# snipsco/sda

Hardware: AMD Instinct MI355X
Metric: share-gen + clerk-sum elements/sec (mod q) (higher is better)
Workload: dtype u64

## Files before the change

sda_amd/csrc/varint_kernels.hip:

```cpp
#include <hip/hip_runtime.h>
#include <stdint.h>

#include "capi_internal.hpp"
#include "drbg_quad.hpp"
#include "kernels.hpp"
#include "modarith.hpp"
#include "sbox_primitives.hpp"

namespace sda {

static constexpr int kVT = 256;
static constexpr int kVals = 8;
static constexpr int kBytes = 16;

__device__ __forceinline__ uint64_t zigzag(int64_t v) { return ((uint64_t)v << 1) ^ (uint64_t)(v >> 63); }
__device__ __forceinline__ uint32_t varint_len(uint64_t zz) {
    const uint32_t x = (64u - (uint32_t)__clzll(zz | 1ull)) + 6u;
    return (x * 37u) >> 8;
}

__device__ __forceinline__ uint32_t block_exscan(uint32_t v, uint32_t* lds_waves, uint32_t* total) {
    const int lane = threadIdx.x & 63, wave = threadIdx.x >> 6;
    uint32_t incl = v;
#pragma unroll
// ... 711 lines not shown
            rs.next_group(sink);
            if (rs.done()) { rs.close(status); live = false; }
        }
        if ((threadIdx.x & 63) == 0) cols[wave] = live ? rs.col : len;
        __syncthreads();
        if (window_flush<kCombWaves>(lo32, hi32, sink, cols, len)) break;
    }
}

static constexpr int kKsStride = 66;
static constexpr int kKsTile = 16 * kKsStride;

struct XSalsaBytes {
    uint32_t key[8], n0, n1;
    uint32_t* ks;
    __device__ __forceinline__ void open(const SboxState& st, uint32_t* tile) {
        const int lane = threadIdx.x & 63;
#pragma unroll
        for (int i = 0; i < 8; ++i) key[i] = st.subkey[i];
        n0 = st.n0; n1 = st.n1;
        ks = tile;
        uint32_t b[16];
        sbx::salsa20_block(b, key, n0, n1, 0);
        if (lane == 0) {
#pragma unroll
            for (int w = 0; w < 16; ++w) ks[w * kKsStride + 64] = b[w];
        }
    }
    __device__ __forceinline__ void begin_group(uint64_t j0) {
        const int lane = threadIdx.x & 63;
        __builtin_amdgcn_fence(__ATOMIC_ACQ_REL, "wavefront");
        __builtin_amdgcn_wave_barrier();
        if (lane < 16) ks[lane * kKsStride] = ks[lane * kKsStride + 64];
        __builtin_amdgcn_fence(__ATOMIC_ACQ_REL, "wavefront");
        __builtin_amdgcn_wave_barrier();
        uint32_t b[16];
        sbx::salsa20_block(b, key, n0, n1, 16 * j0 + 1 + (uint64_t)lane);
#pragma unroll
        for (int w = 0; w < 16; ++w) ks[w * kKsStride + 1 + lane] = b[w];
        __builtin_amdgcn_fence(__ATOMIC_ACQ_REL, "wavefront");
        __builtin_amdgcn_wave_barrier();
    }
    __device__ __forceinline__ void apply(uint4& cur, int d, bool ciphertext) const {
        const uint32_t p = 2u + 64u * (uint32_t)d + (threadIdx.x & 63u);
        const uint32_t* k = ks + (p & 3u) * 4u * kKsStride + (p >> 2);
        if (ciphertext) {
            cur.x ^= k[0]; cur.y ^= k[kKsStride]; cur.z ^= k[2 * kKsStride]; cur.w ^= k[3 * kKsStride];
        }
    }
    __device__ __forceinline__ uint32_t byte_at(uint8_t c, uint64_t m) const {
        const uint64_t sp = m + 32;
        uint32_t b[16];
        sbx::salsa20_block(b, key, n0, n1, sp >> 6);
        uint32_t word = 0;
#pragma unroll
        for (int w = 0; w < 16; ++w) word = ((uint32_t)(sp >> 2) & 15u) == (uint32_t)w ? b[w] : word;
        return (c ^ (word >> (8 * (uint32_t)(sp & 3)))) & 0xFFu;
    }
};

__device__ __forceinline__ bool sealed_row_open(RowStreamT<XSalsaBytes>& rs, const uint8_t* __restrict__ boxes, uint64_t slot,
                                                const uint64_t* __restrict__ row_bytes, uint64_t max_box,
                                                const SboxState* __restrict__ states, uint64_t r, uint64_t len,
                                                uint32_t* __restrict__ status, uint8_t* tile, uint32_t* kstream) {
    const bool lead = (threadIdx.x & 63) == 0;
    const uint64_t have = row_bytes[r];
    if (!(have >= 48 && have <= max_box && have <= slot && !states[r].bad)) return false;
    const uint64_t a = r * slot + 48, b = r * slot + have;
    if (len == 0) { if (a != b && lead) atomicOr(status, SDA_VARINT_ROW_COUNT); return false; }
    if (a == b) { if (lead) atomicOr(status, SDA_VARINT_UNTERMINATED); return false; }
    rs.crypt.open(states[r], kstream);
    if (rs.crypt.byte_at(boxes[b - 1], b - 1 - a) & 0x80u) { if (lead) atomicOr(status, SDA_VARINT_UNTERMINATED); return false; }
    rs.open(boxes, a, b, len, tile);
    return true;
}

template <int kCombWaves>
__global__ __launch_bounds__(kCombWaves * 64) void sealed_stream_combine_kernel(
    const uint8_t* __restrict__ boxes, uint64_t slot, const uint64_t* __restrict__ row_bytes, uint64_t max_box,
    const SboxState* __restrict__ states, uint64_t rows, uint64_t len, uint64_t* __restrict__ acc_lo,
    int64_t* __restrict__ acc_hi, uint32_t* __restrict__ status) {
    __shared__ __attribute__((aligned(16))) uint8_t tiles[kCombWaves][kStreamTile];
    __shared__ uint32_t kstream[kCombWaves][kKsTile];
    __shared__ unsigned long long lo32[kCombWindow], hi32[kCombWindow];
    __shared__ uint64_t cols[kCombWaves];
    const int wave = threadIdx.x >> 6;
    const bool lead = (threadIdx.x & 63) == 0;
    const uint64_t r = (uint64_t)blockIdx.x * kCombWaves + wave;
    for (int i = threadIdx.x; i < kCombWindow; i += kCombWaves * 64) { lo32[i] = 0; hi32[i] = 0; }
    RowStreamT<XSalsaBytes> rs;
    bool live = r < rows && sealed_row_open(rs, boxes, slot, row_bytes, max_box, states, r, len, status, tiles[wave], kstream[wave]);
    WindowSink sink{lo32, hi32, 0, acc_lo, acc_hi};
    __syncthreads();
    for (;;) {
        if (live) {
            rs.next_group(sink);
            if (rs.done()) { rs.close(status); live = false; }
        }
        if (lead) cols[wave] = live ? rs.col : len;
        __syncthreads();
        if (window_flush<kCombWaves>(lo32, hi32, sink, cols, len)) break;
    }
}

static constexpr int kCoefLds = 16;

struct WeightedSink {
    WindowSink win;
    const uint64_t* coef;
    uint32_t k;
    uint64_t batches, m, mu, pinv;
    __device__ __forceinline__ void operator()(uint64_t b, int64_t v) const {
        if (b >= batches) return;
        const uint64_t x = canon_i64(v, m, mu);
        const uint64_t c = b * k;
        for (uint32_t s = 0; s < k; ++s) win(c + s, (int64_t)mont_redc(mul64x64(coef[s], x), m, pinv));
    }
};

template <int kCombWaves, bool kLds>
__global__ __launch_bounds__(kCombWaves * 64) void sealed_stream_weighted_kernel(
    const uint8_t* __restrict__ boxes, uint64_t slot, const uint64_t* __restrict__ row_bytes, uint64_t max_box,
    const SboxState* __restrict__ states, uint64_t rows, uint64_t len, uint64_t first_pos, WeightedJob J,
    uint64_t* __restrict__ acc_lo, int64_t* __restrict__ acc_hi, uint32_t* __restrict__ status) {
    __shared__ __attribute__((aligned(16))) uint8_t tiles[kCombWaves][kStreamTile];
    __shared__ uint32_t kstream[kCombWaves][kKsTile];
    __shared__ unsigned long long lo32[kCombWindow], hi32[kCombWindow];
    __shared__ uint64_t cols[kCombWaves];
    __shared__ uint32_t alive[kCombWaves];
    __shared__ uint64_t coefs[kLds ? kCombWaves : 1][kCoefLds];
    const int wave = __builtin_amdgcn_readfirstlane(threadIdx.x >> 6), lane = threadIdx.x & 63;
    const bool lead = lane == 0;
    const uint64_t r = (uint64_t)blockIdx.x * kCombWaves + wave;
    const uint64_t total = J.batches * J.k;
    for (int i = threadIdx.x; i < kCombWindow; i += kCombWaves * 64) { lo32[i] = 0; hi32[i] = 0; }
    const uint64_t* coef = J.Rt + (first_pos + (r < rows ? r : 0)) * J.k;
    if (kLds) {
        if (r < rows && (uint32_t)lane < J.k) coefs[wave][lane] = coef[lane];
        coef = coefs[wave];
    }
    RowStreamT<XSalsaBytes> rs;
    bool live = r < rows && sealed_row_open(rs, boxes, slot, row_bytes, max_box, states, r, len, status, tiles[wave], kstream[wave]);
    WeightedSink sink{{lo32, hi32, 0, acc_lo, acc_hi}, coef, J.k, J.batches, J.m, J.mu, J.pinv};
    __syncthreads();
    for (;;) {
        if (live) {
            rs.next_group(sink);
            if (rs.done()) { rs.close(status); live = false; }
        }
        if (lead) {
            cols[wave] = live && rs.col < J.batches ? rs.col * J.k : total;
            alive[wave] = live;
        }
        __syncthreads();
        uint32_t any = 0;
#pragma unroll
        for (int w = 0; w < kCombWaves; ++w) any |= alive[w];
        const bool flushed = window_flush<kCombWaves>(lo32, hi32, sink.win, cols, total);
        if (flushed && !any) break;
    }
}

__global__ __launch_bounds__(kVT) void weighted_rows_kernel(const int64_t* __restrict__ shares, uint64_t row_stride, uint32_t rows,
                                                            uint64_t first_pos, WeightedJob J, uint64_t* __restrict__ acc_lo,
                                                            int64_t* __restrict__ acc_hi, uint32_t e_per_group) {
    const uint64_t b = (uint64_t)blockIdx.x * kVT + threadIdx.x;
    if (b >= J.batches) return;
    const uint32_t e0 = blockIdx.y * e_per_group, e1 = e0 + e_per_group < J.k ? e0 + e_per_group : J.k;
    for (uint32_t e = e0; e < e1; ++e) {
        U128 acc{0, 0};
        uint32_t since = 0;
        for (uint32_t c = 0; c < rows; ++c) {
            const uint64_t v = canon_i64(shares[(uint64_t)c * row_stride + b], J.m, J.mu);
            mac128(acc, J.Rt[(first_pos + c) * J.k + e], v);
            if (++since == 4) { mont_acc_condsub(acc, J.m); since = 0; }
        }
        mont_acc_condsub(acc, J.m);
        const uint64_t o = b * J.k + e;
        acc_atomic_add(acc_lo + o, acc_hi + o, mont_redc(acc, J.m, J.pinv), 0);
    }
}

__global__ __launch_bounds__(kVT) void transpose_u64_kernel(const uint64_t* __restrict__ in, uint64_t* __restrict__ out, uint32_t k,
                                                            uint32_t n) {
    const uint64_t i = (uint64_t)blockIdx.x * kVT + threadIdx.x;
    if (i >= (uint64_t)k * n) return;
    const uint64_t pos = i / k, s = i - pos * k;
    out[i] = in[s * n + pos];
}

struct EncXSalsa {
    uint32_t key[8], n0, n1;
    uint32_t* ks;
    uint64_t base;
    __device__ __forceinline__ void fill() {
        const int lane = threadIdx.x & 63;
        __builtin_amdgcn_fence(__ATOMIC_ACQ_REL, "wavefront");
        __builtin_amdgcn_wave_barrier();
        uint32_t b[16];
        sbx::salsa20_block(b, key, n0, n1, base + (uint64_t)lane);
#pragma unroll
        for (int w = 0; w < 16; ++w) ks[w * kKsStride + lane] = b[w];
        __builtin_amdgcn_fence(__ATOMIC_ACQ_REL, "wavefront");
        __builtin_amdgcn_wave_barrier();
    }
    __device__ __forceinline__ void open(const SboxState& st, uint32_t* tile) {
#pragma unroll
        for (int i = 0; i < 8; ++i) key[i] = st.subkey[i];
        n0 = st.n0; n1 = st.n1;
        ks = tile;
        base = 0;
        fill();
    }
    __device__ __forceinline__ bool ends_before(uint64_t unit_end) const { return unit_end + 2 > 4 * (base + 64); }
    __device__ __forceinline__ bool holds(uint64_t u) const { return u + 2 < 4 * (base + 64); }
    __device__ __forceinline__ void refill() { base += 64; fill(); }
    __device__ __forceinline__ void apply(uint4& v, uint64_t u) const {
        const uint32_t p = (uint32_t)(u + 2 - 4 * base);
        const uint32_t* k = ks + (p & 3u) * 4u * kKsStride + (p >> 2);
        v.x ^= k[0]; v.y ^= k[kKsStride]; v.z ^= k[2 * kKsStride]; v.w ^= k[3 * kKsStride];
    }
};

__global__ __launch_bounds__(kStreamWaves * 64) void varint_seal_stream_kernel(VarintRows R, uint8_t* __restrict__ boxes, uint64_t slot,
                                                                               const SboxState* __restrict__ states,
                                                                               uint64_t* __restrict__ msg_bytes) {
    __shared__ __attribute__((aligned(16))) uint8_t tiles[kStreamWaves][kEncTile];
    __shared__ uint32_t kstream[kStreamWaves][kKsTile];
    const int wave = threadIdx.x >> 6;
    const uint64_t r = (uint64_t)blockIdx.x * kStreamWaves + wave;
    if (r >= R.rows) return;
    if (states[r].bad) { if ((threadIdx.x & 63) == 0) msg_bytes[r] = 0; return; }
    EncXSalsa crypt;
    crypt.open(states[r], kstream[wave]);
    LoadValues vals;
    vals.open(R.values + r * R.row_stride, R.len);
    encode_row(vals, R.len, r, boxes + r * slot + 48, tiles[wave], msg_bytes, crypt);
}

template <int ROUNDS>
struct ShareValues {
    static constexpr int kDepth = 1;
    const ShareJob& J;
    const int64_t* __restrict__ sp;
    const uint64_t* __restrict__ row;
    uint64_t stream;
    uint32_t T, draw;
    QuadCol qc;
    __device__ __forceinline__ ShareValues(const ShareJob& J_, uint32_t c, uint64_t p) : J(J_) {
        sp = J.secrets + p * J.secrets_stride;
        stream = J.first_participant + p;
        qc = quad_col(J.key);
        T = J.additive ? J.n - 1 : J.t;
        const uint32_t direct = J.additive ? J.n - 1 : J.direct_rows;
        draw = c < direct ? c : T;
        row = J.additive || c < direct ? nullptr : J.M + (uint64_t)(c - direct) * (J.k + J.t);
    }
    __device__ __forceinline__ void get(int, uint64_t j, int64_t& x, int64_t& y) {
        const uint64_t pair = j * (kEncVals / 2) + (threadIdx.x & 63u);
        const uint64_t b0 = 2 * pair;
        const uint64_t m = J.mod.m, mu = J.mod.mu;
        uint64_t r0, r1;
        if (draw < T) {
            drbg_pair<ROUNDS>(J.key, qc, stream, pair, T, draw, J.mod, r0, r1);
            x = (int64_t)r0; y = (int64_t)r1;
            return;
        }
        if (J.additive) {
            uint64_t s0 = b0 < J.len ? canon_i64(sp[b0], m, mu) : 0;
            uint64_t s1 = b0 + 1 < J.len ? canon_i64(sp[b0 + 1], m, mu) : 0;
            for (uint32_t i = 0; i < T; ++i) {
                drbg_pair<ROUNDS>(J.key, qc, stream, pair, T, i, J.mod, r0, r1);
                s0 = submod(s0, r0, m);
                s1 = submod(s1, r1, m);
            }
            x = (int64_t)s0; y = (int64_t)s1;
            return;
        }
        U128 a0{0, 0}, a1{0, 0};
        uint32_t since = 0;
        const uint64_t e0 = b0 * J.k, e1 = e0 + J.k;
        for (uint32_t i = 0; i < J.k; ++i) {
            const uint64_t v0 = e0 + i < J.len ? canon_i64(sp[e0 + i], m, mu) : 0;
            const uint64_t v1 = e1 + i < J.len ? canon_i64(sp[e1 + i], m, mu) : 0;
            const uint64_t cf = row[i];
            mac128(a0, cf, v0);
            mac128(a1, cf, v1);
            if (++since == 4) { mont_acc_condsub(a0, J.mont.p); mont_acc_condsub(a1, J.mont.p); since = 0; }
        }
        for (uint32_t i = 0; i < T; ++i) {
            drbg_pair<ROUNDS>(J.key, qc, stream, pair, T, i, J.mod, r0, r1);
            const uint64_t cf = row[J.k + i];
            mac128(a0, cf, r0);
            mac128(a1, cf, r1);
            if (++since == 4) { mont_acc_condsub(a0, J.mont.p); mont_acc_condsub(a1, J.mont.p); since = 0; }
        }
        mont_acc_condsub(a0, J.mont.p);
        mont_acc_condsub(a1, J.mont.p);
        x = (int64_t)mont_redc(a0, J.mont.p, J.mont.pinv);
        y = (int64_t)mont_redc(a1, J.mont.p, J.mont.pinv);
    }
};

template <int ROUNDS>
__global__ __launch_bounds__(kStreamWaves * 64) void share_seal_stream_kernel(ShareJob J, uint32_t by_rows, uint8_t* __restrict__ boxes,
                                                                              uint64_t slot, const SboxState* __restrict__ states,
                                                                              uint64_t* __restrict__ msg_bytes) {
    __shared__ __attribute__((aligned(16))) uint8_t tiles[kStreamWaves][kEncTile];
    __shared__ uint32_t kstream[kStreamWaves][kKsTile];
    const int wave = __builtin_amdgcn_readfirstlane(threadIdx.x >> 6);
    uint64_t c, p;
    if (by_rows) {
        const uint64_t r = (uint64_t)blockIdx.x * kStreamWaves + wave;
        c = r / J.participants; p = r - c * J.participants;
    } else {
        const uint32_t groups = (J.n + kStreamWaves - 1) / kStreamWaves;
        p = blockIdx.x / groups;
        c = (uint64_t)(blockIdx.x - p * groups) * kStreamWaves + wave;
    }
    if (c >= J.n || p >= J.participants) return;
    const uint64_t r = c * J.participants + p;
    if (states[r].bad) { if ((threadIdx.x & 63) == 0) msg_bytes[r] = 0; return; }
    EncXSalsa crypt;
    crypt.open(states[r], kstream[wave]);
    ShareValues<ROUNDS> vals(J, (uint32_t)c, p);
    encode_row(vals, J.batches, r, boxes + r * slot + 48, tiles[wave], msg_bytes, crypt);
}

template <int ROUNDS>
struct MaskValues {
    static constexpr int kDepth = 1;
    const MaskJob& J;
    const int64_t* sp;
    int64_t* mp;
    uint64_t stream;
    bool vec;
    QuadCol qc;
    __device__ __forceinline__ MaskValues(const MaskJob& J_, uint64_t p) : J(J_) {
        sp = J.secrets + p * J.secrets_stride;
        mp = J.masked + p * J.masked_stride;
        stream = J.first_participant + p;
        vec = ((((uintptr_t)sp) | ((uintptr_t)mp)) & 15u) == 0;
        qc = quad_col(J.key);
    }
    __device__ __forceinline__ void get(int, uint64_t j, int64_t& x, int64_t& y) {
        typedef long long ll2v __attribute__((ext_vector_type(2)));
        const uint64_t pair = j * (kEncVals / 2) + (threadIdx.x & 63u);
        const uint64_t b0 = 2 * pair;
        const bool two = vec && b0 + 1 < J.len;
        const bool one0 = !two && b0 < J.len, one1 = !two && b0 + 1 < J.len;
        long long s0 = 0, s1 = 0;
        if (two) {
            const ll2v v = __builtin_nontemporal_load(reinterpret_cast<const ll2v*>(sp + b0));
            s0 = v.x; s1 = v.y;
        }
        if (one0) s0 = __builtin_nontemporal_load(reinterpret_cast<const long long*>(sp + b0));
        if (one1) s1 = __builtin_nontemporal_load(reinterpret_cast<const long long*>(sp + b0 + 1));
        __builtin_amdgcn_sched_barrier(0);
        uint64_t r0, r1;
        drbg_pair<ROUNDS>(J.key, qc, stream, pair, 1, 0, J.mod, r0, r1);
        const uint64_t m = J.mod.m, mu = J.mod.mu;
        const long long m0 = (long long)addmod(canon_i64(s0, m, mu), r0, m);
        const long long m1 = (long long)addmod(canon_i64(s1, m, mu), r1, m);
        if (two) {
            ll2v v;
            v.x = m0; v.y = m1;
            __builtin_nontemporal_store(v, reinterpret_cast<ll2v*>(mp + b0));
        }
        if (one0) __builtin_nontemporal_store(m0, reinterpret_cast<long long*>(mp + b0));
        if (one1) __builtin_nontemporal_store(m1, reinterpret_cast<long long*>(mp + b0 + 1));
        x = (int64_t)r0; y = (int64_t)r1;
    }
};

template <int ROUNDS>
__global__ __launch_bounds__(kStreamWaves * 64) void mask_seal_stream_kernel(MaskJob J, uint8_t* __restrict__ boxes, uint64_t slot,
                                                                             const SboxState* __restrict__ states,
                                                                             uint64_t* __restrict__ msg_bytes) {
    __shared__ __attribute__((aligned(16))) uint8_t tiles[kStreamWaves][kEncTile];
    __shared__ uint32_t kstream[kStreamWaves][kKsTile];
    const int wave = __builtin_amdgcn_readfirstlane(threadIdx.x >> 6);
    const uint64_t p = (uint64_t)blockIdx.x * kStreamWaves + wave;
    if (p >= J.participants) return;
    if (states[p].bad) { if ((threadIdx.x & 63) == 0) msg_bytes[p] = 0; return; }
    EncXSalsa crypt;
    crypt.open(states[p], kstream[wave]);
    MaskValues<ROUNDS> vals(J, p);
    encode_row(vals, J.len, p, boxes + p * slot + 48, tiles[wave], msg_bytes, crypt);
}

static constexpr int kSumVals = kVT * kVals;
static constexpr int kSumStage = 64 + kSumVals * 10;
static constexpr int kSumKsBlocks = kSumStage / 64;
static constexpr int kSumKsStride = 17;

size_t sum_seal_blocks(size_t len) { return (size_t)((len + kSumVals - 1) / kSumVals); }

__global__ __launch_bounds__(kVT) void sum_len_kernel(SumRows S, uint32_t* __restrict__ block_bytes) {
    __shared__ uint32_t waves[kVT / 64];
    const uint64_t job = blockIdx.y;
    const uint64_t* lo = S.acc_lo + job * S.len;
    const int64_t* hi = S.acc_hi + job * S.len;
    const uint64_t i0 = (uint64_t)blockIdx.x * kSumVals + threadIdx.x;
    uint32_t sum = 0;
    for (int u = 0; u < kVals; ++u) {
        const uint64_t i = i0 + (uint64_t)u * kVT;
        if (i < S.len) sum += varint_len(zigzag((int64_t)mod_i128(lo[i], hi[i], S.m, S.mu)));
    }
    uint32_t total;
    (void)block_exscan(sum, waves, &total);
    if (threadIdx.x == 0) block_bytes[job * gridDim.x + blockIdx.x] = total;
}

__global__ __launch_bounds__(kVT) void sum_seal_wide_kernel(SumRows S, const uint64_t* __restrict__ block_off, uint8_t* __restrict__ boxes,
                                                            uint64_t slot, const SboxState* __restrict__ states,
                                                            uint64_t* __restrict__ msg_bytes) {
    __shared__ uint32_t waves[kVT / 64];
    __shared__ __attribute__((aligned(16))) uint8_t stage[kSumStage + 16];
    __shared__ uint32_t ks[kSumKsBlocks * kSumKsStride];
    const uint64_t job = blockIdx.y, blk = blockIdx.x, n_blk = gridDim.x;
    const bool last = blk + 1 == n_blk;
    const SboxState& st = states[job];
    if (st.bad) { if (last && threadIdx.x == 0) msg_bytes[job] = 0; return; }
    const uint64_t off = block_off[job * n_blk + blk] - block_off[job * n_blk];
    const uint32_t pad = (uint32_t)((off + 32) & 63u);
    const uint64_t ks0 = (off + 32) >> 6;
    const uint64_t* lo = S.acc_lo + job * S.len;
    const int64_t* hi = S.acc_hi + job * S.len;
    const uint64_t i0 = blk * kSumVals + (uint64_t)threadIdx.x * kVals;
    uint64_t zz[kVals];
    uint32_t ln[kVals];
    uint32_t sum = 0;
    for (int k = 0; k < kVals; ++k) {
        zz[k] = 0; ln[k] = 0;
        if (i0 + k < S.len) {
            zz[k] = zigzag((int64_t)mod_i128(lo[i0 + k], hi[i0 + k], S.m, S.mu));
            ln[k] = varint_len(zz[k]);
            sum += ln[k];
        }
    }
    uint32_t total;
    uint32_t pos = pad + block_exscan(sum, waves, &total);
#pragma unroll
    for (int k = 0; k < kVals; ++k) {
        if (ln[k]) {
            uint64_t n = zz[k];
            for (uint32_t b = 0; b + 1 < ln[k]; ++b) { stage[pos++] = (uint8_t)(0x80u | (n & 0x7Fu)); n >>= 7; }
            stage[pos++] = (uint8_t)n;
        }
    }
    if (total) {
        uint32_t key[8];
#pragma unroll
        for (int i = 0; i < 8; ++i) key[i] = st.subkey[i];
        const uint32_t n_ks = (pad + total + 63u) >> 6;
        for (uint32_t i = threadIdx.x; i < n_ks; i += kVT) {
            uint32_t b[16];
            sbx::salsa20_block(b, key, st.n0, st.n1, ks0 + i);
#pragma unroll
            for (int w = 0; w < 16; ++w) ks[i * kSumKsStride + w] = b[w];
        }
    }
    __syncthreads();
    uint32_t* stage32 = reinterpret_cast<uint32_t*>(stage);
    const uint32_t n_words = total ? (pad + total + 3u) >> 2 : 0u;
    for (uint32_t x = threadIdx.x; x < n_words; x += kVT) stage32[x] ^= ks[(x >> 4) * kSumKsStride + (x & 15u)];
    __syncthreads();
    uint8_t* dst = boxes + job * slot + 48 + off;
    const uint32_t head = (uint32_t)((4u - (uint32_t)((uintptr_t)dst & 3u)) & 3u);
    const uint32_t h = head < total ? head : total;
    if (threadIdx.x < h) dst[threadIdx.x] = stage[pad + threadIdx.x];
    const uint32_t n_dw = (total - h) >> 2;
    uint32_t* dst32 = reinterpret_cast<uint32_t*>(dst + h);
    for (uint32_t d = threadIdx.x; d < n_dw; d += kVT) {
        const uint32_t byte = pad + h + 4u * d;
        const uint32_t w0 = stage32[byte >> 2], w1 = stage32[(byte >> 2) + 1];
        dst32[d] = __builtin_amdgcn_alignbyte(w1, w0, byte & 3u);
    }
    const uint32_t done = h + 4u * n_dw;
    if (threadIdx.x < total - done) dst[done + threadIdx.x] = stage[pad + done + threadIdx.x];
    if (last && threadIdx.x == 0) msg_bytes[job] = off + total;
}

static inline uint64_t vceil(uint64_t a, uint64_t b) { return (a + b - 1) / b; }

size_t varint_encode_blocks(size_t rows, size_t len) { return (size_t)vceil((uint64_t)rows * len, kVT * kVals); }
size_t varint_decode_blocks(size_t n_bytes) { return (size_t)vceil(n_bytes, kVT * kBytes); }

hipError_t launch_varint_lengths(const VarintRows& R, uint32_t* d_block_bytes, hipStream_t s) {
    const size_t nb = varint_encode_blocks(R.rows, R.len);
    if (nb == 0) return hipSuccess;
    if (nb > 0xFFFFFFFFull / kVT) return hipErrorInvalidConfiguration;
    varint_len_kernel<<<dim3((unsigned)nb), dim3(kVT), 0, s>>>(R, d_block_bytes);
    return hipGetLastError();
}

size_t scan_aux_entries(size_t n) { return (n + 1023) / 1024 + 1; }

hipError_t launch_scan_u32(const uint32_t* d_in, uint64_t* d_out, size_t n, uint64_t* d_total, uint64_t* d_aux,
                           hipStream_t s) {
    const size_t m = (n + 1023) / 1024;
    if (m == 0) return hipMemsetAsync(d_total, 0, 8, s);
    if (m > 0xFFFFFFFFull / 1024) return hipErrorInvalidConfiguration;
    scan_chunks_kernel<<<dim3((unsigned)m), dim3(1024), 0, s>>>(d_in, d_out, d_aux, n);
    scan_totals_kernel<<<dim3(1), dim3(1024), 0, s>>>(d_aux, m, d_total);
    scan_add_kernel<<<dim3((unsigned)m), dim3(1024), 0, s>>>(d_out, d_aux, n);
    return hipGetLastError();
}

hipError_t launch_varint_write(const VarintRows& R, const uint64_t* d_block_off, uint8_t* d_out, uint64_t* d_row_offsets,
                               hipStream_t s) {
    const size_t nb = varint_encode_blocks(R.rows, R.len);
    if (nb == 0) return hipSuccess;
    varint_write_kernel<<<dim3((unsigned)nb), dim3(kVT), 0, s>>>(R, d_block_off, d_out, d_row_offsets);
    return hipGetLastError();
}

hipError_t launch_varint_count(const uint8_t* d_bytes, size_t n_bytes, uint32_t* d_block_counts, hipStream_t s) {
    const size_t nb = varint_decode_blocks(n_bytes);
    if (nb == 0) return hipSuccess;
    if (nb > 0xFFFFFFFFull / kVT) return hipErrorInvalidConfiguration;
    varint_count_kernel<<<dim3((unsigned)nb), dim3(kVT), 0, s>>>(d_bytes, n_bytes, d_block_counts);
    return hipGetLastError();
}

hipError_t launch_varint_decode(const uint8_t* d_bytes, size_t n_bytes, const uint64_t* d_block_val_off, size_t rows,
                                size_t len, size_t row_stride, int64_t* d_out, uint32_t* d_status, hipStream_t s) {
    const size_t nb = varint_decode_blocks(n_bytes);
    if (nb == 0) return hipSuccess;
    varint_decode_kernel<<<dim3((unsigned)nb), dim3(kVT), 0, s>>>(d_bytes, n_bytes, d_block_val_off, rows, len, row_stride,
                                                                  d_out, d_status);
    return hipGetLastError();
}

hipError_t launch_varint_stream_decode(const uint8_t* d_bytes, size_t n_bytes, const RowRanges& d_offsets, size_t rows,
                                       size_t len, size_t row_stride, int64_t* d_out, uint32_t* d_status, hipStream_t s) {
    if (rows == 0) return hipSuccess;
    varint_stream_decode_kernel<<<dim3((unsigned)vceil(rows, kStreamWaves)), dim3(kStreamWaves * 64), 0, s>>>(
        d_bytes, n_bytes, d_offsets, rows, len, row_stride, d_out, d_status);
    return hipGetLastError();
}

hipError_t launch_varint_stream_encode(const VarintRows& R, uint8_t* d_out, size_t slot_bytes, uint64_t* d_row_bytes,
                                       hipStream_t s) {
    if (R.rows == 0) return hipSuccess;
    varint_stream_encode_kernel<<<dim3((unsigned)vceil(R.rows, kStreamWaves)), dim3(kStreamWaves * 64), residency_pad_bytes(knob(KNOB_WIRE_WG_PER_CU), 8192), s>>>(
        R, d_out, slot_bytes, d_row_bytes);
    return hipGetLastError();
}

hipError_t launch_varint_seal_stream(const VarintRows& R, uint8_t* d_boxes, size_t slot_bytes, const SboxState* d_states,
                                     uint64_t* d_msg_bytes, hipStream_t s) {
    if (R.rows == 0) return hipSuccess;
    const uint64_t groups = vceil(R.rows, kStreamWaves);
    if (groups > 0x7FFFFFFFull) return hipErrorInvalidConfiguration;
    varint_seal_stream_kernel<<<dim3((unsigned)groups), dim3(kStreamWaves * 64), 0, s>>>(R, d_boxes, slot_bytes, d_states, d_msg_bytes);
    return hipGetLastError();
}

static bool sum_grid(const SumRows& S, dim3* grid) {
    const uint64_t nb = sum_seal_blocks(S.len);
    if (S.jobs > 65535 || nb * S.jobs > 0xFFFFFFFFull / kVT) return false;
    *grid = dim3((unsigned)nb, (unsigned)S.jobs);
    return true;
}

hipError_t launch_sum_lengths(const SumRows& S, uint32_t* d_block_bytes, hipStream_t s) {
    if (S.jobs == 0 || S.len == 0) return hipSuccess;
    dim3 grid;
    if (!sum_grid(S, &grid)) return hipErrorInvalidConfiguration;
    sum_len_kernel<<<grid, dim3(kVT), 0, s>>>(S, d_block_bytes);
    return hipGetLastError();
}

hipError_t launch_sum_seal_wide(const SumRows& S, const uint64_t* d_block_off, uint8_t* d_boxes, size_t slot_bytes,
                                const SboxState* d_states, uint64_t* d_msg_bytes, hipStream_t s) {
    if (S.jobs == 0) return hipSuccess;
    if (S.len == 0) return hipMemsetAsync(d_msg_bytes, 0, S.jobs * sizeof(uint64_t), s);
    dim3 grid;
    if (!sum_grid(S, &grid)) return hipErrorInvalidConfiguration;
    sum_seal_wide_kernel<<<grid, dim3(kVT), 0, s>>>(S, d_block_off, d_boxes, slot_bytes, d_states, d_msg_bytes);
    return hipGetLastError();
}

hipError_t launch_share_seal_stream(const ShareJob& J, int rounds, uint8_t* d_boxes, size_t slot_bytes, const SboxState* d_states,
                                    uint64_t* d_msg_bytes, hipStream_t s) {
    if (J.participants == 0 || J.n == 0) return hipSuccess;
    const bool by_rows = knob(KNOB_GENSEAL_BY_ROWS) != 0;
    const uint64_t groups = by_rows ? vceil((uint64_t)J.n * J.participants, kStreamWaves) : vceil(J.n, kStreamWaves) * (uint64_t)J.participants;
    if (groups > 0x7FFFFFFFull) return hipErrorInvalidConfiguration;
    const dim3 grid((unsigned)groups), block(kStreamWaves * 64);
    switch (rounds) {
        case 20: share_seal_stream_kernel<20><<<grid, block, 0, s>>>(J, by_rows, d_boxes, slot_bytes, d_states, d_msg_bytes); break;
        case 12: share_seal_stream_kernel<12><<<grid, block, 0, s>>>(J, by_rows, d_boxes, slot_bytes, d_states, d_msg_bytes); break;
        case 8: share_seal_stream_kernel<8><<<grid, block, 0, s>>>(J, by_rows, d_boxes, slot_bytes, d_states, d_msg_bytes); break;
        default: return hipErrorInvalidValue;
    }
    return hipGetLastError();
}

hipError_t launch_mask_seal_stream(const MaskJob& J, int rounds, uint8_t* d_boxes, size_t slot_bytes, const SboxState* d_states,
                                   uint64_t* d_msg_bytes, hipStream_t s) {
    if (J.participants == 0) return hipSuccess;
    const uint64_t groups = vceil(J.participants, kStreamWaves);
    if (groups > 0x7FFFFFFFull) return hipErrorInvalidConfiguration;
    const dim3 grid((unsigned)groups), block(kStreamWaves * 64);
    switch (rounds) {
        case 20: mask_seal_stream_kernel<20><<<grid, block, 0, s>>>(J, d_boxes, slot_bytes, d_states, d_msg_bytes); break;
        case 12: mask_seal_stream_kernel<12><<<grid, block, 0, s>>>(J, d_boxes, slot_bytes, d_states, d_msg_bytes); break;
        case 8: mask_seal_stream_kernel<8><<<grid, block, 0, s>>>(J, d_boxes, slot_bytes, d_states, d_msg_bytes); break;
        default: return hipErrorInvalidValue;
    }
    return hipGetLastError();
}

hipError_t launch_varint_stream_combine(const uint8_t* d_bytes, size_t n_bytes, const RowRanges& d_offsets, size_t jobs,
                                        size_t rows_per_job, size_t len, uint64_t* d_acc_lo, int64_t* d_acc_hi,
                                        uint32_t* d_status, hipStream_t s) {
    if (jobs == 0 || rows_per_job == 0 || len == 0) return hipSuccess;
    const bool wide = vceil(rows_per_job, 16) * jobs >= 512;
    const uint64_t groups = vceil(rows_per_job, wide ? 16 : 8);
    if (groups * jobs > 0x7FFFFFFFull) return hipErrorInvalidConfiguration;
    if (wide)
        varint_stream_combine_kernel<16><<<dim3((unsigned)(groups * jobs)), dim3(16 * 64), residency_pad_bytes(knob(KNOB_WIRE_WG_PER_CU), 49152), s>>>(
            d_bytes, n_bytes, d_offsets, rows_per_job, groups, len, d_acc_lo, d_acc_hi, d_status);
    else
        varint_stream_combine_kernel<8><<<dim3((unsigned)(groups * jobs)), dim3(8 * 64), 0, s>>>(
            d_bytes, n_bytes, d_offsets, rows_per_job, groups, len, d_acc_lo, d_acc_hi, d_status);
    return hipGetLastError();
}

hipError_t launch_sealed_stream_combine(const uint8_t* d_boxes, size_t slot, const uint64_t* d_row_bytes, size_t rows,
                                        size_t max_box_bytes, const SboxState* d_states, size_t len, uint64_t* d_acc_lo,
                                        int64_t* d_acc_hi, uint32_t* d_status, hipStream_t s, int* waves) {
    if (waves) *waves = 0;
    if (rows == 0) return hipSuccess;
    const bool wide = knob(KNOB_SEALED_WAVES) == 16;
    const uint64_t groups = vceil(rows, wide ? 16 : 8);
    if (groups > 0x7FFFFFFFull) return hipErrorInvalidConfiguration;
    if (waves) *waves = wide ? 16 : 8;
    if (wide)
        sealed_stream_combine_kernel<16><<<dim3((unsigned)groups), dim3(16 * 64), 0, s>>>(d_boxes, slot, d_row_bytes, max_box_bytes, d_states,
                                                                                       rows, len, d_acc_lo, d_acc_hi, d_status);
    else
        sealed_stream_combine_kernel<8><<<dim3((unsigned)groups), dim3(8 * 64), 0, s>>>(d_boxes, slot, d_row_bytes, max_box_bytes, d_states,
                                                                                     rows, len, d_acc_lo, d_acc_hi, d_status);
    return hipGetLastError();
}

hipError_t launch_sealed_stream_weighted(const uint8_t* d_boxes, size_t slot, const uint64_t* d_row_bytes, size_t rows,
                                         size_t max_box_bytes, const SboxState* d_states, size_t len, size_t first_pos,
                                         const WeightedJob& J, uint64_t* d_acc_lo, int64_t* d_acc_hi, uint32_t* d_status,
                                         hipStream_t s) {
    if (rows == 0) return hipSuccess;
    const uint64_t groups = vceil(rows, 8);
    if (groups > 0x7FFFFFFFull) return hipErrorInvalidConfiguration;
    if (J.k <= (uint32_t)kCoefLds)
        sealed_stream_weighted_kernel<8, true><<<dim3((unsigned)groups), dim3(8 * 64), 0, s>>>(
            d_boxes, slot, d_row_bytes, max_box_bytes, d_states, rows, len, first_pos, J, d_acc_lo, d_acc_hi, d_status);
    else
        sealed_stream_weighted_kernel<8, false><<<dim3((unsigned)groups), dim3(8 * 64), 0, s>>>(
            d_boxes, slot, d_row_bytes, max_box_bytes, d_states, rows, len, first_pos, J, d_acc_lo, d_acc_hi, d_status);
    return hipGetLastError();
}

hipError_t launch_weighted_rows(const int64_t* d_shares, size_t row_stride, size_t rows, size_t first_pos, const WeightedJob& J,
                                uint64_t* d_acc_lo, int64_t* d_acc_hi, hipStream_t s) {
    if (rows == 0 || J.batches == 0) return hipSuccess;
    const uint64_t blocks = vceil(J.batches, kVT);
    if (blocks > 0x7FFFFFFFull || rows > 0xFFFFFFFFull) return hipErrorInvalidConfiguration;
    uint64_t groups = blocks < 2048 ? vceil(2048, blocks) : 1;
    if (groups > J.k) groups = J.k;
    const uint32_t e_per_group = (uint32_t)vceil(J.k, groups);
    groups = vceil(J.k, e_per_group);
    weighted_rows_kernel<<<dim3((unsigned)blocks, (unsigned)groups), dim3(kVT), 0, s>>>(d_shares, row_stride, (uint32_t)rows, first_pos, J,
                                                                                      d_acc_lo, d_acc_hi, e_per_group);
    return hipGetLastError();
}

hipError_t launch_transpose_u64(const uint64_t* d_in, uint64_t* d_out, uint32_t k, uint32_t n, hipStream_t s) {
    const uint64_t blocks = vceil((uint64_t)k * n, kVT);
    if (blocks == 0) return hipSuccess;
    if (blocks > 0x7FFFFFFFull) return hipErrorInvalidConfiguration;
    transpose_u64_kernel<<<dim3((unsigned)blocks), dim3(kVT), 0, s>>>(d_in, d_out, k, n);
    return hipGetLastError();
}

hipError_t launch_varint_rowcheck(const uint8_t* d_bytes, size_t n_bytes, const uint64_t* d_offsets, size_t rows, size_t len,
                                  const uint64_t* d_block_val_off, uint32_t* d_status, hipStream_t s) {
    if (rows == 0) return hipSuccess;
    varint_rowcheck_kernel<<<dim3((unsigned)vceil(rows, kVT / 64)), dim3(kVT), 0, s>>>(d_bytes, n_bytes, d_offsets, rows, len,
                                                                                   d_block_val_off, d_status);
    return hipGetLastError();
}

}
```

Baseline: 116.9 billion.

## Share secrets and DRBG draws across waves via LDS in share-seal kernel

Adds a share-seal kernel variant in which waves of a workgroup (same participant, different share columns) cooperatively load and canonicalise secrets and generate DRBG randomness once into double-buffered dynamic LDS. Each wave then forms its share from the shared inputs instead of recomputing all draws itself. This removes redundant per-column DRBG work and secret loads, at the cost of block barriers each step, LDS pressure that can lower occupancy, and idle waves being forced to stay in sync. It is selected by default when the LDS budget fits and the by-rows knob is off.

After: 116.5 billion. Within noise of the previous version (-0.4%).

```diff
diff --git a/sda_amd/csrc/varint_kernels.hip b/sda_amd/csrc/varint_kernels.hip
--- a/sda_amd/csrc/varint_kernels.hip
+++ b/sda_amd/csrc/varint_kernels.hip
@@ -1037,6 +1037,125 @@
     }
 };
 
+static constexpr int kShareRow = kEncVals + 2;
+static constexpr size_t kLdsPerCu = 160 * 1024;
+
+extern __shared__ __attribute__((aligned(16))) uint64_t share_inputs[];
+
+template <int ROUNDS, int WAVES>
+struct SharedShareValues {
+    static constexpr int kDepth = 1;
+    const ShareJob& J;
+    const int64_t* __restrict__ sp;
+    const uint64_t* __restrict__ row;
+    uint64_t stream, n_steps;
+    uint32_t T, draw, terms;
+    uint32_t wave, piece0;
+    int64_t pre0, pre1;
+    QuadCol qc;
+    __device__ __forceinline__ SharedShareValues(const ShareJob& J_, uint32_t c, uint64_t p, uint32_t wave_) : J(J_), wave(wave_) {
+        sp = J.secrets + p * J.secrets_stride;
+        stream = J.first_participant + p;
+        qc = quad_col(J.key);
+        T = J.additive ? J.n - 1 : J.t;
+        terms = J.k + T;
+        const uint32_t direct = J.additive ? J.n - 1 : J.direct_rows;
+        draw = c < direct ? c : T;
+        row = J.additive || c < direct ? nullptr : J.M + (uint64_t)(c - direct) * terms;
+        n_steps = (J.batches + kEncVals - 1) / kEncVals;
+        piece0 = WAVES - 1 - wave;
+        pre0 = pre1 = 0;
+        if (n_steps) {
+            load_first(0);
+            produce(0);
+        }
+        sync();
+    }
+    __device__ __forceinline__ static void sync() {
+        __builtin_amdgcn_fence(__ATOMIC_RELEASE, "workgroup");
+        __builtin_amdgcn_s_barrier();
+        __builtin_amdgcn_fence(__ATOMIC_ACQUIRE, "workgroup");
+    }
+    __device__ __forceinline__ int64_t secret_at(uint64_t e) const { return e < J.len ? sp[e] : 0; }
+    __device__ __forceinline__ void put_secret(uint32_t buf, uint32_t e, uint64_t v) const {
+        const uint32_t b = e / J.k, i = e - b * J.k;
+        share_inputs[buf + i * kShareRow + b] = v;
+    }
+    __device__ __forceinline__ void load_first(uint64_t j) {
+        if (piece0 >= J.k) return;
+        const uint64_t e = j * kEncVals * J.k + piece0 * kEncVals + (threadIdx.x & 63u);
+        pre0 = secret_at(e);
+        pre1 = secret_at(e + 64);
+    }
+    __device__ __forceinline__ void produce(uint64_t j) {
+        const uint32_t lane = threadIdx.x & 63u;
+        const uint32_t buf = (uint32_t)(j & 1) * terms * kShareRow;
+        const uint64_t m = J.mod.m, mu = J.mod.mu;
+        const uint64_t e0 = j * kEncVals * J.k;
+        if (piece0 < J.k) {
+            const uint32_t e = piece0 * kEncVals + lane;
+            put_secret(buf, e, e0 + e < J.len ? canon_i64(pre0, m, mu) : 0);
+            put_secret(buf, e + 64, e0 + e + 64 < J.len ? canon_i64(pre1, m, mu) : 0);
+            load_first(j + 1);
+        }
+        for (uint32_t piece = piece0 + WAVES; piece < J.k; piece += WAVES) {
+            const uint32_t e = piece * kEncVals + lane;
+            const int64_t s0 = secret_at(e0 + e), s1 = secret_at(e0 + e + 64);
+            put_secret(buf, e, e0 + e < J.len ? canon_i64(s0, m, mu) : 0);
+            put_secret(buf, e + 64, e0 + e + 64 < J.len ? canon_i64(s1, m, mu) : 0);
+        }
+        const uint64_t pair = j * (kEncVals / 2) + lane;
+        for (uint32_t i = wave; i < T; i += WAVES) {
+            uint64_t r0, r1;
+            drbg_pair<ROUNDS>(J.key, qc, stream, pair, T, i, J.mod, r0, r1);
+            *reinterpret_cast<ulonglong2*>(&share_inputs[buf + (J.k + i) * kShareRow + 2 * lane]) = make_ulonglong2(r0, r1);
+        }
+    }
+    __device__ __forceinline__ ulonglong2 input(uint32_t buf, uint32_t i) const {
+        return *reinterpret_cast<const ulonglong2*>(&share_inputs[buf + i * kShareRow + 2 * (threadIdx.x & 63u)]);
+    }
+    __device__ __forceinline__ void skip(uint64_t j) {
+        if (j + 1 < n_steps) produce(j + 1);
+        sync();
+    }
+    __device__ __forceinline__ void skip_row() {
+        for (uint64_t j = 0; j < n_steps; ++j) skip(j);
+    }
+    __device__ __forceinline__ void get(int, uint64_t j, int64_t& x, int64_t& y) {
+        if (j + 1 < n_steps) produce(j + 1);
+        const uint32_t buf = (uint32_t)(j & 1) * terms * kShareRow;
+        if (draw < T) {
+            const ulonglong2 d = input(buf, J.k + draw);
+            x = (int64_t)d.x; y = (int64_t)d.y;
+        } else if (J.additive) {
+            const uint64_t m = J.mod.m;
+            const ulonglong2 s = input(buf, 0);
+            uint64_t s0 = s.x, s1 = s.y;
+            for (uint32_t i = 0; i < T; ++i) {
+                const ulonglong2 d = input(buf, 1 + i);
+                s0 = submod(s0, d.x, m);
+                s1 = submod(s1, d.y, m);
+            }
+            x = (int64_t)s0; y = (int64_t)s1;
+        } else {
+            U128 a0{0, 0}, a1{0, 0};
+            uint32_t since = 0;
+            for (uint32_t i = 0; i < terms; ++i) {
+                const ulonglong2 v = input(buf, i);
+                const uint64_t cf = row[i];
+                mac128(a0, cf, v.x);
+                mac128(a1, cf, v.y);
+                if (++since == 4) { mont_acc_condsub(a0, J.mont.p); mont_acc_condsub(a1, J.mont.p); since = 0; }
+            }
+            mont_acc_condsub(a0, J.mont.p);
+            mont_acc_condsub(a1, J.mont.p);
+            x = (int64_t)mont_redc(a0, J.mont.p, J.mont.pinv);
+            y = (int64_t)mont_redc(a1, J.mont.p, J.mont.pinv);
+        }
+        sync();
+    }
+};
+
 template <int ROUNDS>
 __global__ __launch_bounds__(kStreamWaves * 64) void share_seal_stream_kernel(ShareJob J, uint32_t by_rows, uint8_t* __restrict__ boxes,
                                                                               uint64_t slot, const SboxState* __restrict__ states,
@@ -1060,6 +1179,33 @@
     crypt.open(states[r], kstream[wave]);
     ShareValues<ROUNDS> vals(J, (uint32_t)c, p);
     encode_row(vals, J.batches, r, boxes + r * slot + 48, tiles[wave], msg_bytes, crypt);
+}
+
+template <int ROUNDS, int WAVES>
+__global__ __launch_bounds__(WAVES * 64) void share_seal_stream_kernel(ShareJob J, uint8_t* __restrict__ boxes, uint64_t slot,
+                                                                       const SboxState* __restrict__ states,
+                                                                       uint64_t* __restrict__ msg_bytes) {
+    __shared__ __attribute__((aligned(16))) uint8_t tiles[WAVES][kEncTile];
+    __shared__ uint32_t kstream[WAVES][kKsTile];
+    const int wave = __builtin_amdgcn_readfirstlane(threadIdx.x >> 6);
+    const uint32_t groups = (J.n + WAVES - 1) / WAVES;
+    const uint64_t p = blockIdx.x / groups;
+    const uint64_t c = (uint64_t)(blockIdx.x - p * groups) * WAVES + wave;
+    const uint64_t r = c * J.participants + p;
+    bool live = c < J.n;
+    if (live && states[r].bad) {
+        if ((threadIdx.x & 63) == 0) msg_bytes[r] = 0;
+        live = false;
+    }
+    live = __builtin_amdgcn_readfirstlane(live);
+    SharedShareValues<ROUNDS, WAVES> vals(J, (uint32_t)c, p, (uint32_t)wave);
+    if (live) {
+        EncXSalsa crypt;
+        crypt.open(states[r], kstream[wave]);
+        encode_row(vals, J.batches, r, boxes + r * slot + 48, tiles[wave], msg_bytes, crypt);
+    } else {
+        vals.skip_row();
+    }
 }
 
 template <int ROUNDS>
@@ -1318,10 +1464,52 @@
     return hipGetLastError();
 }
 
+template <int ROUNDS, int WAVES>
+static bool launch_share_seal_waves(const ShareJob& J, uint8_t* d_boxes, size_t slot_bytes, const SboxState* d_states,
+                                    uint64_t* d_msg_bytes, hipStream_t s, hipError_t* err) {
+    const size_t input_bytes = 2 * (size_t)(J.k + (J.additive ? J.n - 1 : J.t)) * kShareRow * 8;
+    const size_t tile_bytes = (size_t)WAVES * (kEncTile + kKsTile * 4);
+    if (2 * (input_bytes + tile_bytes) > kLdsPerCu) return false;
+    const uint64_t wgs = vceil(J.n, WAVES) * (uint64_t)J.participants;
+    const auto kern = share_seal_stream_kernel<ROUNDS, WAVES>;
+    *err = hipSuccess;
+    if (wgs > 0x7FFFFFFFull) {
+        *err = hipErrorInvalidConfiguration;
+    } else {
+        if (input_bytes + tile_bytes > 48 * 1024)
+            *err = hipFuncSetAttribute(reinterpret_cast<const void*>(kern), hipFuncAttributeMaxDynamicSharedMemorySize, (int)input_bytes);
+        if (*err == hipSuccess) {
+            kern<<<dim3((unsigned)wgs), dim3(WAVES * 64), input_bytes, s>>>(J, d_boxes, slot_bytes, d_states, d_msg_bytes);
+            *err = hipGetLastError();
+        }
+    }
+    return true;
+}
+
+template <int ROUNDS>
+static bool launch_share_seal_shared(const ShareJob& J, uint8_t* d_boxes, size_t slot_bytes, const SboxState* d_states,
+                                     uint64_t* d_msg_bytes, hipStream_t s, hipError_t* err) {
+    const bool wide = vceil(J.n, 8) * 8 <= vceil(J.n, 4) * 4;
+    if (wide && launch_share_seal_waves<ROUNDS, 8>(J, d_boxes, slot_bytes, d_states, d_msg_bytes, s, err)) return true;
+    if (launch_share_seal_waves<ROUNDS, 4>(J, d_boxes, slot_bytes, d_states, d_msg_bytes, s, err)) return true;
+    return !wide && launch_share_seal_waves<ROUNDS, 8>(J, d_boxes, slot_bytes, d_states, d_msg_bytes, s, err);
+}
+
 hipError_t launch_share_seal_stream(const ShareJob& J, int rounds, uint8_t* d_boxes, size_t slot_bytes, const SboxState* d_states,
                                     uint64_t* d_msg_bytes, hipStream_t s) {
     if (J.participants == 0 || J.n == 0) return hipSuccess;
     const bool by_rows = knob(KNOB_GENSEAL_BY_ROWS) != 0;
+    if (!by_rows) {
+        hipError_t err = hipSuccess;
+        bool done = false;
+        switch (rounds) {
+            case 20: done = launch_share_seal_shared<20>(J, d_boxes, slot_bytes, d_states, d_msg_bytes, s, &err); break;
+            case 12: done = launch_share_seal_shared<12>(J, d_boxes, slot_bytes, d_states, d_msg_bytes, s, &err); break;
+            case 8: done = launch_share_seal_shared<8>(J, d_boxes, slot_bytes, d_states, d_msg_bytes, s, &err); break;
+            default: return hipErrorInvalidValue;
+        }
+        if (done) return err;
+    }
     const uint64_t groups = by_rows ? vceil((uint64_t)J.n * J.participants, kStreamWaves) : vceil(J.n, kStreamWaves) * (uint64_t)J.participants;
     if (groups > 0x7FFFFFFFull) return hipErrorInvalidConfiguration;
     const dim3 grid((unsigned)groups), block(kStreamWaves * 64);
```
